# hendraet/synthesis-in-style

Measured on NVIDIA B200. Metric: labelled image pairs/sec at 256^2, higher is better.
Workload: dtype bf16x3 (3-term bf16 split, fp32 accumulate)

## Files before the change

### synthesis_in_style_b200/csrc/modconv_tc.cu

```cuda
#include <cuda.h>
#include <cstring>
#include "common.cuh"
#include "kernels.h"
#include "modconv_tc.h"

namespace sis {

using bf16 = __nv_bfloat16;

__device__ __forceinline__ uint32_t smem_u32(const void* p) { return (uint32_t)__cvta_generic_to_shared(p); }

__device__ __forceinline__ bool elect_one() {
    uint32_t pred;
    asm volatile("{\n\t.reg .pred P;\n\telect.sync _|P, 0xffffffff;\n\tselp.u32 %0, 1, 0, P;\n\t}" : "=r"(pred));
    return pred != 0;
}

__device__ __forceinline__ void mbar_init(uint64_t* bar, uint32_t count) {
    asm volatile("mbarrier.init.shared::cta.b64 [%0], %1;" ::"r"(smem_u32(bar)), "r"(count) : "memory");
}
__device__ __forceinline__ void mbar_expect_tx(uint64_t* bar, uint32_t bytes, uint32_t pred = 1u) {
    asm volatile("{\n\t.reg .pred q;\n\tsetp.ne.b32 q, %2, 0;\n\t@q mbarrier.arrive.expect_tx.shared::cta.b64 _, [%0], %1;\n\t}"
                 ::"r"(smem_u32(bar)), "r"(bytes), "r"(pred) : "memory");
}
// ... 671 lines not shown
template <int BN, int BK, bool UP4>
__global__ void __launch_bounds__(TC_THREADS, 1)
modconv_tc_halo_rw_kernel(const __grid_constant__ TcMaps maps, const __grid_constant__ TcKernelArgs a) {
    using Cfg = TcHaloRwCfg<BN, BK, UP4>;
    constexpr int NA = Cfg::NA, ROW = Cfg::ROW;
    extern __shared__ uint8_t smem_raw[];
    uint8_t* smem_w = (uint8_t*)(((uintptr_t)smem_raw + 1023) & ~(uintptr_t)1023);
    uint8_t* smem_a = smem_w + Cfg::W_BYTES;
    uint64_t* bars = (uint64_t*)(smem_a + NA * Cfg::A_STAGE);
    uint64_t* afull_bar = bars;
    uint64_t* aempty_bar = bars + NA;
    uint64_t* tfull_bar = bars + 2 * NA;
    uint64_t* tempty_bar = tfull_bar + 2;
    uint64_t* wfull_bar = tempty_bar + 2;
    uint32_t* tmem_ptr_smem = (uint32_t*)(wfull_bar + 1);

    const int warp = __shfl_sync(0xffffffffu, (int)(threadIdx.x >> 5), 0), lane = threadIdx.x & 31;
    const int unit0 = (int)blockIdx.x, unit_stride = (int)gridDim.x;
    if (warp == 0 && lane == 0) {
        tma_prefetch_desc(&maps.a[0][0]); tma_prefetch_desc(&maps.a[0][1]);
        tma_prefetch_desc(&maps.w[0]); tma_prefetch_desc(&maps.w[1]);
        for (int i = 0; i < NA; ++i) { mbar_init(&afull_bar[i], 1); mbar_init(&aempty_bar[i], 1); }
        for (int i = 0; i < 2; ++i) { mbar_init(&tfull_bar[i], 1); mbar_init(&tempty_bar[i], TC_EPI_WARPS); }
        mbar_init(wfull_bar, 1);
        asm volatile("fence.mbarrier_init.release.cluster;" ::: "memory");
    }
    if (warp == 1) {
        asm volatile("tcgen05.alloc.cta_group::1.sync.aligned.shared::cta.b32 [%0], %1;" ::"r"(smem_u32(tmem_ptr_smem)), "r"((uint32_t)Cfg::TMEM_COLS) : "memory");
        asm volatile("tcgen05.relinquish_alloc_permit.cta_group::1.sync.aligned;" ::: "memory");
    }
    tc_fence_before();
    __syncthreads();
    tc_fence_after();
    const uint32_t tmem_base = *tmem_ptr_smem;
    const TcSubProblem& s = a.sub[0];

    if (warp == 0) {
        if (elect_one()) {
            mbar_expect_tx(wfull_bar, Cfg::W_BYTES);
            for (int tap = 0; tap < 9; ++tap) {
                tma_load_3d(&maps.w[0], wfull_bar, smem_w + tap * Cfg::W_TAP, 0, 0, s.widx[tap]);
                tma_load_3d(&maps.w[1], wfull_bar, smem_w + tap * Cfg::W_TAP + Cfg::W_TILE, 0, 0, s.widx[tap]);
            }
        }
        __syncwarp();
        int as = 0; uint32_t aphase = 0;
        for (int t = unit0; t < a.total_tiles; t += unit_stride) {
            const TileCoord c = decode_tile<BN, true, 1>(a, t, 0);
            mbar_wait(&aempty_bar[as], aphase ^ 1, a.error, 0x500 + as);
            uint8_t* sa = smem_a + as * Cfg::A_STAGE;
            if (elect_one()) {
                mbar_expect_tx(&afull_bar[as], 2 * Cfg::A_BYTES);
                tma_load_4d(&maps.a[0][0], &afull_bar[as], sa, 0, c.x0 - 1, c.y0 - 1, c.b0);
                tma_load_4d(&maps.a[0][1], &afull_bar[as], sa + Cfg::A_PAD, 0, c.x0 - 1, c.y0 - 1, c.b0);
            }
            __syncwarp();
            if (++as == NA) { as = 0; aphase ^= 1; }
        }
    } else if (warp == 1) {
        constexpr uint32_t idesc = (1u << 4) | (1u << 7) | (1u << 10) | ((uint32_t)(BN >> 3) << 17) | ((uint32_t)(BM >> 4) << 24);
        int as = 0; uint32_t aphase = 0;
        int acc = 0; uint32_t acc_phase = 0;
        mbar_wait(wfull_bar, 0, a.error, 0x700);
        const uint32_t sw0 = smem_u32(smem_w);
        for (int t = unit0; t < a.total_tiles; t += unit_stride) {
            mbar_wait(&tempty_bar[acc], acc_phase ^ 1, a.error, 0x200 + acc);
            mbar_wait(&afull_bar[as], aphase, a.error, 0x600 + as);
            tc_fence_after();
            const uint32_t d_tile = tmem_base + (uint32_t)(acc * Cfg::ACC_COLS);
            const uint32_t sa = smem_u32(smem_a + as * Cfg::A_STAGE);
            if (elect_one()) {
                uint32_t started = 0;
#pragma unroll 1
                for (int tap = 0; tap < 9; ++tap) {
                    const uint32_t aoff = (uint32_t)(((s.dy[tap] + 1) * HALO_W + (s.dx[tap] + 1)) * ROW);
                    const uint64_t d_ah = make_halo_desc<ROW>(sa + aoff), d_al = make_halo_desc<ROW>(sa + Cfg::A_PAD + aoff);
                    const uint32_t sb = sw0 + (uint32_t)(tap * Cfg::W_TAP);
                    const uint64_t d_bh = make_smem_desc<ROW>(sb), d_bl = make_smem_desc<ROW>(sb + Cfg::W_TILE);
                    const int ph = UP4 ? s.phase[tap] : 0;
                    const uint32_t d_tmem = d_tile + (uint32_t)(ph * BN);
                    const uint32_t fresh = UP4 ? (((started >> ph) & 1u) ^ 1u) : (tap ? 0u : 1u);
                    started |= 1u << ph;
#pragma unroll
                    for (int k = 0; k < BK / UMMA_K; ++k) {
                        const uint64_t koff = (uint64_t)((k * UMMA_K * 2) >> 4);
                        umma_bf16(d_tmem, d_ah + koff, d_bh + koff, idesc, (fresh && k == 0) ? 0u : 1u);
                        umma_bf16(d_tmem, d_ah + koff, d_bl + koff, idesc, 1u);
                        umma_bf16(d_tmem, d_al + koff, d_bh + koff, idesc, 1u);
                    }
                }
                umma_commit(&aempty_bar[as]);
                umma_commit(&tfull_bar[acc]);
            }
            __syncwarp();
            if (++as == NA) { as = 0; aphase ^= 1; }
            if (++acc == 2) { acc = 0; acc_phase ^= 1; }
        }
    } else {
        tc_epilogue<BN, true, 1, UP4>(a, tfull_bar, tempty_bar, tmem_base, 0, warp, lane, unit0, unit_stride);
    }
    tc_fence_before();
    __syncthreads();
    if (warp == 1) {
        __syncwarp();
        tc_fence_after();
        asm volatile("tcgen05.dealloc.cta_group::1.sync.aligned.b32 %0, %1;" ::"r"(tmem_base), "r"((uint32_t)Cfg::TMEM_COLS) : "memory");
    }
}

constexpr int HT_TH = 32, HT_TW = 8, HT_W = HT_TW + 2, HT_H = HT_TH + 2, HT_BK = 32, HT_N = HT_TH * HT_TW;
struct TcHaloTCfg {
    static constexpr int ROW = HT_BK * 2;
    static constexpr int A_BYTES = HT_H * HT_W * ROW;
    static constexpr int A_PAD = (A_BYTES + 1023) / 1024 * 1024;
    static constexpr int A_STAGE = 2 * A_PAD;
    static constexpr int NA = 2;
    static constexpr int W_TILE_BYTES = 128 * ROW;
    static constexpr int W_STAGE = 2 * W_TILE_BYTES;
    static constexpr int NW = 8;
    static constexpr int SMEM_BYTES = NA * A_STAGE + NW * W_STAGE + 1024 + 512;
    static constexpr int TMEM_COLS = 512;
};

__device__ __forceinline__ uint64_t make_halo_t_desc(uint32_t saddr) {
    uint64_t d = 0;
    d |= (uint64_t)((saddr >> 4) & 0x3FFF);
    d |= (uint64_t)1 << 16;
    d |= (uint64_t)((HT_W * TcHaloTCfg::ROW) >> 4) << 32;
    d |= (uint64_t)1 << 46;
    d |= (uint64_t)4 << 61;
    return d;
}

__global__ void __launch_bounds__(TC_THREADS, 1)
modconv_tc_halo_t_kernel(const __grid_constant__ TcMaps maps, const __grid_constant__ TcKernelArgs a) {
    using Cfg = TcHaloTCfg;
    constexpr int NA = Cfg::NA, NW = Cfg::NW, BK = HT_BK;
    extern __shared__ uint8_t smem_raw[];
    uint8_t* smem = (uint8_t*)(((uintptr_t)smem_raw + 1023) & ~(uintptr_t)1023);
    uint8_t* smem_w = smem + NA * Cfg::A_STAGE;
    uint64_t* bars = (uint64_t*)(smem_w + NW * Cfg::W_STAGE);
    uint64_t* full_bar = bars;
    uint64_t* empty_bar = bars + NW;
    uint64_t* afull_bar = bars + 2 * NW;
    uint64_t* aempty_bar = bars + 2 * NW + NA;
    uint64_t* tfull_bar = bars + 2 * NW + 2 * NA;
    uint64_t* tempty_bar = tfull_bar + 2;
    uint32_t* tmem_ptr_smem = (uint32_t*)(tempty_bar + 2);

    const int warp = __shfl_sync(0xffffffffu, (int)(threadIdx.x >> 5), 0), lane = threadIdx.x & 31;
    const int tiles_x = a.sub[0].ow / HT_TW, tiles_y = a.sub[0].oh / HT_TH;
    const int m_tiles = a.batch * tiles_y * tiles_x;
    const int per = a.nsub;

    if (warp == 0 && lane == 0) {
        tma_prefetch_desc(&maps.a[0][0]); tma_prefetch_desc(&maps.a[0][1]);
        tma_prefetch_desc(&maps.w[0]); tma_prefetch_desc(&maps.w[1]);
        for (int i = 0; i < NW; ++i) { mbar_init(&full_bar[i], 1); mbar_init(&empty_bar[i], 1); }
        for (int i = 0; i < NA; ++i) { mbar_init(&afull_bar[i], 1); mbar_init(&aempty_bar[i], 1); }
        for (int i = 0; i < 2; ++i) { mbar_init(&tfull_bar[i], 1); mbar_init(&tempty_bar[i], TC_EPI_WARPS); }
        asm volatile("fence.mbarrier_init.release.cluster;" ::: "memory");
    }
    if (warp == 1) {
        asm volatile("tcgen05.alloc.cta_group::1.sync.aligned.shared::cta.b32 [%0], %1;" ::"r"(smem_u32(tmem_ptr_smem)), "r"((uint32_t)Cfg::TMEM_COLS) : "memory");
        asm volatile("tcgen05.relinquish_alloc_permit.cta_group::1.sync.aligned;" ::: "memory");
    }
    tc_fence_before();
    __syncthreads();
    tc_fence_after();
    const uint32_t tmem_base = *tmem_ptr_smem;

    if (warp == 0) {
        {
            int as = 0; uint32_t aphase = 0;
            int ws = 0; uint32_t wphase = 0;
            for (int t = blockIdx.x; t < a.total_tiles; t += gridDim.x) {
                const int rt = t % (m_tiles * per), n0 = (t / (m_tiles * per)) * 128;
                const int m = rt / per;
                const TcSubProblem& s = a.sub[per == 1 ? 0 : ((rt % per) + m) & 3];
                const int x0 = (m % tiles_x) * HT_TW, y0 = ((m / tiles_x) % tiles_y) * HT_TH, b = m / (tiles_x * tiles_y);
                for (int kc = 0; kc < a.kchunks; ++kc) {
                    mbar_wait(&aempty_bar[as], aphase ^ 1, a.error, 0x500 + as);
                    uint8_t* sa = smem + as * Cfg::A_STAGE;
                    if (elect_one()) {
                        mbar_expect_tx(&afull_bar[as], 2 * Cfg::A_BYTES);
                        tma_load_4d(&maps.a[0][0], &afull_bar[as], sa, kc * BK, x0 - 1, y0 - 1, b);
                        tma_load_4d(&maps.a[0][1], &afull_bar[as], sa + Cfg::A_PAD, kc * BK, x0 - 1, y0 - 1, b);
                    }
                    __syncwarp();
                    if (++as == NA) { as = 0; aphase ^= 1; }
                    for (int tap = 0; tap < s.ntaps; ++tap) {
                        mbar_wait(&empty_bar[ws], wphase ^ 1, a.error, 0x100 + ws);
                        uint8_t* sw = smem_w + ws * Cfg::W_STAGE;
                        if (elect_one()) {
                            mbar_expect_tx(&full_bar[ws], Cfg::W_STAGE);
                            tma_load_3d(&maps.w[0], &full_bar[ws], sw, kc * BK, n0, s.widx[tap]);
                            tma_load_3d(&maps.w[1], &full_bar[ws], sw + Cfg::W_TILE_BYTES, kc * BK, n0, s.widx[tap]);
                        }
                        __syncwarp();
                        if (++ws == NW) { ws = 0; wphase ^= 1; }
                    }
                }
            }
        }
    } else if (warp == 1) {
        {
            constexpr uint32_t idesc = (1u << 4) | (1u << 7) | (1u << 10) | ((uint32_t)(HT_N >> 3) << 17) | ((uint32_t)(128 >> 4) << 24);
            int as = 0; uint32_t aphase = 0;
            int ws = 0; uint32_t wphase = 0;
            int acc = 0; uint32_t acc_phase = 0;
            for (int t = blockIdx.x; t < a.total_tiles; t += gridDim.x) {
                const int rt = t % (m_tiles * per);
                const TcSubProblem& s = a.sub[per == 1 ? 0 : ((rt % per) + rt / per) & 3];
                mbar_wait(&tempty_bar[acc], acc_phase ^ 1, a.error, 0x200 + acc);
                tc_fence_after();
                const uint32_t d_tmem = tmem_base + (uint32_t)(acc * HT_N);
                for (int kc = 0; kc < a.kchunks; ++kc) {
                    mbar_wait(&afull_bar[as], aphase, a.error, 0x600 + as);
                    const uint32_t sa = smem_u32(smem + as * Cfg::A_STAGE);
                    for (int tap = 0; tap < s.ntaps; ++tap) {
                        mbar_wait(&full_bar[ws], wphase, a.error, 0x300 + ws);
                        tc_fence_after();
                        const uint32_t xoff = (uint32_t)(((s.dy[tap] + 1) * HT_W + (s.dx[tap] + 1)) * Cfg::ROW);
                        const uint64_t d_xh = make_halo_t_desc(sa + xoff), d_xl = make_halo_t_desc(sa + Cfg::A_PAD + xoff);
                        const uint32_t sw = smem_u32(smem_w + ws * Cfg::W_STAGE);
                        const uint64_t d_wh = make_smem_desc<Cfg::ROW>(sw), d_wl = make_smem_desc<Cfg::ROW>(sw + Cfg::W_TILE_BYTES);
                        if (elect_one()) {
#pragma unroll
                            for (int k = 0; k < BK / UMMA_K; ++k) {
                                const uint64_t koff = (uint64_t)((k * UMMA_K * 2) >> 4);
                                umma_bf16(d_tmem, d_wh + koff, d_xh + koff, idesc, (kc | tap | k) ? 1u : 0u);
                                umma_bf16(d_tmem, d_wl + koff, d_xh + koff, idesc, 1u);
                                umma_bf16(d_tmem, d_wh + koff, d_xl + koff, idesc, 1u);
                            }
                            umma_commit(&empty_bar[ws]);
                            if (tap == s.ntaps - 1) {
                                umma_commit(&aempty_bar[as]);
                                if (kc == a.kchunks - 1) umma_commit(&tfull_bar[acc]);
                            }
                        }
                        __syncwarp();
                        if (++ws == NW) { ws = 0; wphase ^= 1; }
                    }
                    if (++as == NA) { as = 0; aphase ^= 1; }
                }
                if (++acc == 2) { acc = 0; acc_phase ^= 1; }
            }
        }
    } else {
        const int quarter = warp & 3;
        const int chalf = (warp - 2) >> 2;
        int acc = 0; uint32_t acc_phase = 0;
        for (int t = blockIdx.x; t < a.total_tiles; t += gridDim.x) {
            const int rt = t % (m_tiles * per), n0 = (t / (m_tiles * per)) * 128;
            const int m = rt / per;
            const TcSubProblem& s = a.sub[per == 1 ? 0 : ((rt % per) + m) & 3];
            const int x0 = (m % tiles_x) * HT_TW, y0 = ((m / tiles_x) % tiles_y) * HT_TH, b = m / (tiles_x * tiles_y);
            const int ch = n0 + quarter * 32 + lane;
            const float d = __ldg(a.demod + (int64_t)b * a.cout + ch);
            const float bias = a.bias ? __ldg(a.bias + ch) : 0.0f;
            const float sn = a.s_next ? __ldg(a.s_next + (int64_t)b * a.cout + ch) : 0.0f;
            float* plane = a.out_f32 + ((int64_t)b * a.cout + ch) * ((int64_t)a.out_h * a.out_w);
            const float* nzp = a.noise ? a.noise + (int64_t)b * a.noise_bstride : nullptr;
            mbar_wait(&tfull_bar[acc], acc_phase, a.error, 0x400 + acc);
            tc_fence_after();
            const uint32_t taddr = tmem_base + ((uint32_t)(quarter * 32) << 16) + (uint32_t)(acc * HT_N);
#pragma unroll 1
            for (int c0 = chalf * 32; c0 < HT_N; c0 += 64) {
                uint32_t r[32];
                tmem_ld_32x32(taddr + (uint32_t)c0, r);
                tmem_ld_wait();
                if (a.mode == 1) {
#pragma unroll
                    for (int rr = 0; rr < 4; ++rr) {
                        const int oy = (y0 + c0 / HT_TW + rr) * s.ostride + s.ooff_y;
                        float* row = a.out_f32 + (((int64_t)b * a.out_h + oy) * a.out_w + x0 * s.ostride + s.ooff_x) * a.cout + ch;
#pragma unroll
                        for (int j = 0; j < 8; ++j) row[(int64_t)j * s.ostride * a.cout] = __fmul_rn(__uint_as_float(r[rr * 8 + j]), d);
                    }
                    continue;
                }
#pragma unroll
                for (int rr = 0; rr < 4; ++rr) {
                    const int y = y0 + c0 / HT_TW + rr;
                    float nz[8] = {0.f, 0.f, 0.f, 0.f, 0.f, 0.f, 0.f, 0.f};
                    if (nzp) {
                        const float4 n0v = __ldg(reinterpret_cast<const float4*>(nzp + (int64_t)y * a.out_w + x0));
                        const float4 n1v = __ldg(reinterpret_cast<const float4*>(nzp + (int64_t)y * a.out_w + x0) + 1);
                        nz[0] = n0v.x; nz[1] = n0v.y; nz[2] = n0v.z; nz[3] = n0v.w; nz[4] = n1v.x; nz[5] = n1v.y; nz[6] = n1v.z; nz[7] = n1v.w;
                    }
                    float v[8];
#pragma unroll
                    for (int j = 0; j < 8; ++j) {
                        float x = __fmul_rn(__uint_as_float(r[rr * 8 + j]), d);
                        x = __fadd_rn(x, __fmul_rn(a.noise_w, nz[j]));
                        if (a.bias) x = __fadd_rn(x, bias);
                        if (a.act) x = lrelu_scale(x, 0.2f, 1.41421356237309504880f);
                        v[j] = x;
                    }
                    float4* dst = reinterpret_cast<float4*>(plane + (int64_t)y * a.out_w + x0);
                    dst[0] = make_float4(v[0], v[1], v[2], v[3]);
                    dst[1] = make_float4(v[4], v[5], v[6], v[7]);
                    if (a.s_next) {
                        const int64_t off = (((int64_t)b * a.out_h + y) * a.out_w + x0) * a.cout + (ch & ~1);
#pragma unroll
                        for (int j = 0; j < 8; ++j) {
                            const float xs = __fmul_rn(v[j], sn);
                            const float other = __shfl_xor_sync(0xffffffffu, xs, 1);
                            if ((j & 1) == (lane & 1)) {
                                const float c0v = (lane & 1) ? other : xs, c1v = (lane & 1) ? xs : other;
                                const bf16 h0 = __float2bfloat16_rn(c0v), h1 = __float2bfloat16_rn(c1v);
                                const bf16 l0 = __float2bfloat16_rn(c0v - __bfloat162float(h0)), l1 = __float2bfloat16_rn(c1v - __bfloat162float(h1));
                                *reinterpret_cast<uint32_t*>(a.next_hi + off + (int64_t)j * a.cout) =
                                    (uint32_t)__bfloat16_as_ushort(h0) | ((uint32_t)__bfloat16_as_ushort(h1) << 16);
                                *reinterpret_cast<uint32_t*>(a.next_lo + off + (int64_t)j * a.cout) =
                                    (uint32_t)__bfloat16_as_ushort(l0) | ((uint32_t)__bfloat16_as_ushort(l1) << 16);
                            }
                        }
                    }
                }
            }
            tc_fence_before();
            __syncwarp();
            if (lane == 0) mbar_arrive(&tempty_bar[acc]);
            if (++acc == 2) { acc = 0; acc_phase ^= 1; }
        }
    }
    tc_fence_before();
    __syncthreads();
    if (warp == 1) {
        __syncwarp();
        tc_fence_after();
        asm volatile("tcgen05.dealloc.cta_group::1.sync.aligned.b32 %0, %1;" ::"r"(tmem_base), "r"((uint32_t)Cfg::TMEM_COLS) : "memory");
    }
}

struct BlurSplitArgs {
    const float* in; int IH, IW;
    float* out_f32; int OH, OW, C, batch;
    const float* blur_k; const float* noise; int64_t noise_bstride; float noise_w; const float* bias;
    const float* s_next; bf16* next_hi; bf16* next_lo;
    int act;
};
constexpr int BS_TH = 8, BS_IH = BS_TH + 3;
template <int CB> struct BlurGeo {
    static constexpr int LPG = CB / 2;
    static constexpr int GROUPS = 32 / LPG;
    static constexpr int TW = 8 * GROUPS * 2;
    static constexpr int IW = TW + 3;
    static constexpr int OPITCH = BS_TH * TW + 1;
    static constexpr int SMEM = BS_IH * IW * CB * 4;
    static_assert(CB * OPITCH * 4 <= SMEM, "the transposed output must fit in the input tile");
};

using u64 = unsigned long long;
__device__ __forceinline__ float2 ffma2(float2 a, float2 b, float2 c) {
    float2 d;
    asm("fma.rn.f32x2 %0, %1, %2, %3;" : "=l"(reinterpret_cast<u64&>(d)) : "l"(reinterpret_cast<u64&>(a)), "l"(reinterpret_cast<u64&>(b)), "l"(reinterpret_cast<u64&>(c)));
    return d;
}
__device__ __forceinline__ float2 fmul2(float2 a, float2 b) {
    float2 d;
    asm("mul.rn.f32x2 %0, %1, %2;" : "=l"(reinterpret_cast<u64&>(d)) : "l"(reinterpret_cast<u64&>(a)), "l"(reinterpret_cast<u64&>(b)));
    return d;
}
__device__ __forceinline__ float2 fadd2(float2 a, float2 b) {
    float2 d;
    asm("add.rn.f32x2 %0, %1, %2;" : "=l"(reinterpret_cast<u64&>(d)) : "l"(reinterpret_cast<u64&>(a)), "l"(reinterpret_cast<u64&>(b)));
    return d;
}
__device__ __forceinline__ float2 splat2(float v) { return make_float2(v, v); }
__device__ __forceinline__ float2 lds_f2(uint32_t addr) {
    float2 v;
    asm volatile("ld.shared.v2.f32 {%0, %1}, [%2];" : "=f"(v.x), "=f"(v.y) : "r"(addr));
    return v;
}
__device__ __forceinline__ float lds_f1(uint32_t addr) {
    float v;
    asm volatile("ld.shared.f32 %0, [%1];" : "=f"(v) : "r"(addr));
    return v;
}
__device__ __forceinline__ void sts_f1(uint32_t addr, float v) { asm volatile("st.shared.f32 [%0], %1;" ::"r"(addr), "f"(v) : "memory"); }

template <bool SEP, int CB>
__global__ void __launch_bounds__(256, 2) blur_act_split_kernel(BlurSplitArgs a, const __grid_constant__ CUtensorMap in_map) {
    using G = BlurGeo<CB>;
    constexpr int TW = G::TW, IW = G::IW, LPG = G::LPG, OPITCH = G::OPITCH, TILE_BYTES = G::SMEM;
    extern __shared__ __align__(128) float stile_raw[];
    __shared__ float sk[16], skx[4], sky[4];
    __shared__ float snz[BS_TH * TW];
    __shared__ uint64_t tma_bar[2];
    float* const ring0 = (float*)(((uintptr_t)stile_raw + 127) & ~(uintptr_t)127);
    const int tid = threadIdx.x, lane = tid & 31, warp = tid >> 5;
    const int grp = lane / LPG, cl = lane - grp * LPG;
    if (tid < 16) sk[tid] = a.blur_k[(3 - tid / 4) * 4 + (3 - tid % 4)];
    __syncthreads();
    if (tid < 4) { sky[tid] = sk[tid * 4]; skx[tid] = SEP ? sk[tid] / sk[0] : 0.0f; }
    const int tiles_x = (a.OW + TW - 1) / TW, tiles_y = (a.OH + BS_TH - 1) / BS_TH;
    const int cgroups = (a.C + CB - 1) / CB;
    const int64_t total = (int64_t)a.batch * tiles_y * tiles_x * cgroups;
    auto tile_coords = [&](int64_t tile, int& b, int& y0, int& x0, int& c0) {
        const int cg = (int)(tile % cgroups);
        int64_t r = tile / cgroups;
        const int tx = (int)(r % tiles_x); r /= tiles_x;
        const int ty = (int)(r % tiles_y);
        b = (int)(r / tiles_y); y0 = ty * BS_TH; x0 = tx * TW; c0 = cg * CB;
    };
    if (tid == 0) {
        mbar_init(&tma_bar[0], 1); mbar_init(&tma_bar[1], 1);
        asm volatile("fence.mbarrier_init.release.cluster;" ::: "memory");
        if ((int64_t)blockIdx.x < total) {
            int b, y0, x0, c0;
            tile_coords(blockIdx.x, b, y0, x0, c0);
            mbar_expect_tx(&tma_bar[0], TILE_BYTES);
            tma_load_4d(&in_map, &tma_bar[0], ring0, c0, x0 - 1, y0 - 1, b);
        }
    }
    int it = 0;
    for (int64_t tile = blockIdx.x; tile < total; tile += gridDim.x, ++it) {
        int b, y0, x0, c0;
        tile_coords(tile, b, y0, x0, c0);
        float* const stile = ring0 + (it & 1) * (TILE_BYTES / 4);
        const uint32_t stile_u32 = smem_u32(stile);
        __syncthreads();
        if (tid == 0 && tile + gridDim.x < total) {
            int nb, ny0, nx0, nc0;
            tile_coords(tile + gridDim.x, nb, ny0, nx0, nc0);
            asm volatile("fence.proxy.async.shared::cta;" ::: "memory");
            mbar_expect_tx(&tma_bar[(it + 1) & 1], TILE_BYTES);
            tma_load_4d(&in_map, &tma_bar[(it + 1) & 1], ring0 + ((it + 1) & 1) * (TILE_BYTES / 4), nc0, nx0 - 1, ny0 - 1, nb);
        }
        if (tid < BS_TH * TW) {
            const int oy = y0 + tid / TW, ox = x0 + tid % TW;
            snz[tid] = (a.noise && oy < a.OH && ox < a.OW) ? a.noise_w * __ldg(a.noise + (int64_t)b * a.noise_bstride + (int64_t)oy * a.OW + ox) : 0.0f;
        }
        mbar_wait(&tma_bar[it & 1], (uint32_t)((it >> 1) & 1), nullptr, 0);
        __syncthreads();

        float2 res[2][BS_TH];
        const int px = (warp * G::GROUPS + grp) * 2;
        const uint32_t in_base = stile_u32 + (uint32_t)(px * LPG + cl) * 8u;
        {
            const bool chok = c0 + 2 * cl < a.C;
            const float2 bias = (chok && a.bias) ? *reinterpret_cast<const float2*>(a.bias + c0 + 2 * cl) : make_float2(0.f, 0.f);
            const float2 sn = (a.s_next && chok) ? *reinterpret_cast<const float2*>(a.s_next + (int64_t)b * a.C + c0 + 2 * cl) : make_float2(0.f, 0.f);
            const bool colok0 = chok && x0 + px < a.OW, colok1 = chok && x0 + px + 1 < a.OW;
            const int64_t off0 = (((int64_t)b * a.OH + y0) * a.OW + x0 + px) * a.C + c0 + 2 * cl;
            __nv_bfloat162* ph = reinterpret_cast<__nv_bfloat162*>(a.next_hi + off0);
            __nv_bfloat162* pl = reinterpret_cast<__nv_bfloat162*>(a.next_lo + off0);
            const int c2 = a.C >> 1;
            const int64_t rs2 = ((int64_t)a.OW * a.C) >> 1;
            const bool st0 = a.s_next != nullptr && colok0, st1 = a.s_next != nullptr && colok1;
            float2 win[2][4][SEP ? 1 : 4];
#pragma unroll
            for (int rr = 0; rr < BS_IH; ++rr) {
                float2 in5[5];
#pragma unroll
                for (int j = 0; j < 5; ++j) in5[j] = lds_f2(in_base + (uint32_t)((rr * IW + j) * LPG) * 8u);
#pragma unroll
                for (int cx = 0; cx < 2; ++cx) {
#pragma unroll
                    for (int ky = 0; ky < 3; ++ky)
#pragma unroll
                        for (int kx = 0; kx < (SEP ? 1 : 4); ++kx) win[cx][ky][kx] = win[cx][ky + 1][kx];
                    if (SEP) {
                        float2 h = make_float2(0.f, 0.f);
#pragma unroll
                        for (int kx = 0; kx < 4; ++kx) h = ffma2(in5[cx + kx], splat2(skx[kx]), h);
                        win[cx][3][0] = h;
                    } else {
#pragma unroll
                        for (int kx = 0; kx < 4; ++kx) win[cx][3][kx] = in5[cx + kx];
                    }
                }
                if (rr >= 3) {
                    const int py = rr - 3;
                    const bool rowok = y0 + py < a.OH;
#pragma unroll
// ... 320 lines not shown
    for (int ky = py; ky < 3; ky += 2)
        for (int kx = px; kx < 3; kx += 2) {
            s.dy[s.ntaps] = (short)(y0 - ky / 2); s.dx[s.ntaps] = (short)(x0 - kx / 2);
            s.widx[s.ntaps] = (signed char)(ky * 3 + kx); s.phase[s.ntaps] = (signed char)(py * 2 + px); s.ntaps++;
        }
}

static void set_im2col_runs(TcSubProblem& s, int batch) {
    s.m_tiles = (int)ceil_div64((int64_t)batch * s.oh * s.ow, BM);
    s.base_dy = s.dy[0]; s.base_dx = s.dx[0];
    for (int t = 1; t < s.ntaps; ++t) { s.base_dy = std::min<int>(s.base_dy, s.dy[t]); s.base_dx = std::min<int>(s.base_dx, s.dx[t]); }
}

static TcKernelArgs conv_args(const TcWorkspace& ws, const TcConvCall& call, int BK) {
    TcKernelArgs a;
    memset(&a, 0, sizeof(a));
    const int H = call.res_in;
    a.batch = call.batch; a.cin = call.cin; a.cout = call.cout; a.kchunks = call.cin / BK; a.b_tiles = call.batch;
    a.demod = call.demod; a.error = ws.d_error;
    if (call.up) {
        a.mode = 1;
        a.out_f32 = call.upconv_tmp; a.out_h = 2 * H + 1; a.out_w = 2 * H + 1;
    } else {
        a.mode = 0; a.act = call.act ? 1 : 0;
        a.noise = call.noise; a.noise_bstride = call.noise_bstride; a.noise_w = call.noise_w; a.bias = call.bias;
        a.out_f32 = call.out_f32; a.out_h = H; a.out_w = H;
        a.s_next = call.s_next; a.next_hi = (bf16*)ws.a_hi[call.out_slot]; a.next_lo = (bf16*)ws.a_lo[call.out_slot];
    }
    return a;
}

template <auto Kernel, int SMEM_BYTES, int CG = 1>
static int launch_persistent(const TcMaps& maps, const TcKernelArgs& a, cudaStream_t stream) {
    static bool configured = false;
    if (!configured) {
        SIS_CHECK_CUDA(cudaFuncSetAttribute(Kernel, cudaFuncAttributeMaxDynamicSharedMemorySize, SMEM_BYTES));
        configured = true;
    }
    cudaLaunchConfig_t cfg;
    memset(&cfg, 0, sizeof(cfg));
    cfg.gridDim = dim3(a.total_tiles * CG < kNumSMs ? a.total_tiles * CG : kNumSMs);
    cfg.blockDim = dim3(TC_THREADS); cfg.dynamicSmemBytes = SMEM_BYTES; cfg.stream = stream;
    cudaLaunchAttribute attr[1];
    attr[0].id = cudaLaunchAttributeClusterDimension;
    attr[0].val.clusterDim.x = CG; attr[0].val.clusterDim.y = 1; attr[0].val.clusterDim.z = 1;
    cfg.attrs = attr; cfg.numAttrs = 1;
    SIS_CHECK_CUDA(cudaLaunchKernelEx(&cfg, Kernel, maps, a));
    SIS_CHECK_LAUNCH();
    return SIS_OK;
}

template <int BK, int CG>
static int launch_tc(int BN, const TcMaps& maps, const TcKernelArgs& a, cudaStream_t stream) {
    if (BN == 256) return launch_persistent<modconv_tc_kernel<256, BK, CG>, TcCfg<256, BK, CG>::SMEM_BYTES, CG>(maps, a, stream);
    if (BN == 128) return launch_persistent<modconv_tc_kernel<128, BK, CG>, TcCfg<128, BK, CG>::SMEM_BYTES, CG>(maps, a, stream);
    if (BN == 64) return launch_persistent<modconv_tc_kernel<64, BK, CG>, TcCfg<64, BK, CG>::SMEM_BYTES, CG>(maps, a, stream);
    if constexpr (CG == 1) {
        if (BN == 32) return launch_persistent<modconv_tc_kernel<32, BK, 1>, TcCfg<32, BK, 1>::SMEM_BYTES>(maps, a, stream);
    }
    set_error("tc_modconv: no per-tap kernel for BN %d with CG %d", BN, CG);
    return SIS_ERR_UNSUPPORTED;
}

template <int CG>
static int launch_tc_halo(int BN, int BK, const TcMaps& maps, const TcKernelArgs& a, cudaStream_t stream) {
    if (BK == 32) {
        if (BN == 64) return launch_persistent<modconv_tc_halo_kernel<64, CG, 32, false>, TcHaloCfg<64, CG, 32, false>::SMEM_BYTES, CG>(maps, a, stream);
        if constexpr (CG == 1) {
            if (BN == 32) return launch_persistent<modconv_tc_halo_kernel<32, 1, 32, false>, TcHaloCfg<32, 1, 32, false>::SMEM_BYTES>(maps, a, stream);
        }
    } else {
        if (BN == 256) return launch_persistent<modconv_tc_halo_kernel<256, CG, 64, false>, TcHaloCfg<256, CG, 64, false>::SMEM_BYTES, CG>(maps, a, stream);
        if (BN == 128) return launch_persistent<modconv_tc_halo_kernel<128, CG, 64, false>, TcHaloCfg<128, CG, 64, false>::SMEM_BYTES, CG>(maps, a, stream);
        if (BN == 64) return launch_persistent<modconv_tc_halo_kernel<64, CG, 64, false>, TcHaloCfg<64, CG, 64, false>::SMEM_BYTES, CG>(maps, a, stream);
        if constexpr (CG == 1) {
            if (BN == 32) return launch_persistent<modconv_tc_halo_kernel<32, 1, 64, false>, TcHaloCfg<32, 1, 64, false>::SMEM_BYTES>(maps, a, stream);
        }
    }
    set_error("tc_modconv: no halo kernel for BN %d, BK %d with CG %d", BN, BK, CG);
    return SIS_ERR_UNSUPPORTED;
}

static int launch_tc_halo_up4(int BN, int BK, int CG, const TcMaps& maps, const TcKernelArgs& a, cudaStream_t stream) {
    if (BN == 64 && CG == 2) {
        if (BK == 64) return launch_persistent<modconv_tc_halo_kernel<64, 2, 64, true>, TcHaloCfg<64, 2, 64, true>::SMEM_BYTES, 2>(maps, a, stream);
        return launch_persistent<modconv_tc_halo_kernel<64, 2, 32, true>, TcHaloCfg<64, 2, 32, true>::SMEM_BYTES, 2>(maps, a, stream);
    }
    if (BN == 64) {
        if (BK == 64) return launch_persistent<modconv_tc_halo_kernel<64, 1, 64, true>, TcHaloCfg<64, 1, 64, true>::SMEM_BYTES>(maps, a, stream);
        return launch_persistent<modconv_tc_halo_kernel<64, 1, 32, true>, TcHaloCfg<64, 1, 32, true>::SMEM_BYTES>(maps, a, stream);
    }
    if (BK == 64) return launch_persistent<modconv_tc_halo_kernel<32, 1, 64, true>, TcHaloCfg<32, 1, 64, true>::SMEM_BYTES>(maps, a, stream);
    return launch_persistent<modconv_tc_halo_kernel<32, 1, 32, true>, TcHaloCfg<32, 1, 32, true>::SMEM_BYTES>(maps, a, stream);
}

template <int CB>
static int launch_blur_split(const BlurSplitArgs& bs, bool sep, cudaStream_t stream) {
    using G = BlurGeo<CB>;
    static int blocks_per_sm[2] = {0, 0};
    const size_t smem = 2 * (size_t)G::SMEM + 128;
    auto kern = sep ? blur_act_split_kernel<true, CB> : blur_act_split_kernel<false, CB>;
    int& bps = blocks_per_sm[sep ? 1 : 0];
    if (!bps) {
        SIS_CHECK_CUDA(cudaFuncSetAttribute(kern, cudaFuncAttributeMaxDynamicSharedMemorySize, (int)smem));
        SIS_CHECK_CUDA(cudaOccupancyMaxActiveBlocksPerMultiprocessor(&bps, kern, 256, smem));
        if (bps < 1) bps = 1;
    }
    CUtensorMap in_map;
    memset(&in_map, 0, sizeof(in_map));
    const uint64_t dims[4] = {(uint64_t)bs.C, (uint64_t)bs.IW, (uint64_t)bs.IH, (uint64_t)bs.batch};
    const uint32_t box[4] = {(uint32_t)CB, (uint32_t)G::IW, (uint32_t)BS_IH, 1};
    SIS_PROPAGATE(make_map_f32(&in_map, bs.in, 4, dims, box));
    const int64_t total = (int64_t)bs.batch * ceil_div(bs.OH, BS_TH) * ceil_div(bs.OW, G::TW) * ceil_div(bs.C, CB);
    const int grid = (int)std::min<int64_t>(total, (int64_t)kNumSMs * bps);
    ProfScope prof(PROF_BLUR_SPLIT, stream);
    kern<<<grid, 256, smem, stream>>>(bs, in_map);
    SIS_CHECK_LAUNCH();
    return SIS_OK;
}

static int tc_blur_after_upconv(TcWorkspace& ws, const TcConvCall& call, cudaStream_t stream) {
    const int B = call.batch, H = call.res_in;
    BlurSplitArgs bs;
    bs.in = call.upconv_tmp; bs.IH = 2 * H + 1; bs.IW = 2 * H + 1;
    bs.out_f32 = call.out_f32; bs.OH = call.res_out; bs.OW = call.res_out; bs.C = call.cout; bs.batch = B;
    bs.blur_k = call.blur_k; bs.noise = call.noise; bs.noise_bstride = call.noise_bstride; bs.noise_w = call.noise_w; bs.bias = call.bias;
    bs.s_next = call.s_next; bs.next_hi = (bf16*)ws.a_hi[call.out_slot]; bs.next_lo = (bf16*)ws.a_lo[call.out_slot];
    bs.act = call.act ? 1 : 0;
    SIS_REQUIRE(bs.C % 32 == 0, "tc_modconv: the blur pass needs Cout %% 32 == 0 (got %d)", bs.C);
    if (bs.C % 64 != 0 && bs.OW >= 32) return launch_blur_split<32>(bs, call.blur_separable, stream);
    return launch_blur_split<64>(bs, call.blur_separable, stream);
}

int tc_modconv(TcWorkspace& ws, const TcConvWeights& w, const TcConvCall& call, cudaStream_t stream) {
    const int conv_cat = call.cout <= 64 ? PROF_CONV_TC_NARROW : PROF_CONV_TC;
    SIS_REQUIRE(w.hi && w.cin == call.cin && w.cout == call.cout, "tc_modconv: weights not packed for this layer");
    const int B = call.batch, H = call.res_in;
    if (!call.up && call.cout == 128 && call.cin % HT_BK == 0 && H % HT_TH == 0) {
        TcKernelArgs a = conv_args(ws, call, HT_BK);
        a.nsub = 1;
        TcSubProblem& s = a.sub[0];
        set_conv_taps(s);
        s.oh = H; s.ow = H; s.ostride = 1;
        a.total_tiles = B * (H / HT_TH) * (H / HT_TW);
        TcMaps maps;
        memset(&maps, 0, sizeof(maps));
        SIS_PROPAGATE(make_halo_maps(maps, ws, call, HT_BK, HT_W, HT_H));
        SIS_PROPAGATE(make_weight_maps(maps, w.hi, w.lo, call.cin, call.cout, 9, HT_BK, 128));
        ProfScope prof(conv_cat, stream);
        return launch_persistent<modconv_tc_halo_t_kernel, TcHaloTCfg::SMEM_BYTES>(maps, a, stream);
    }
    if (call.up && call.cout == 128 && call.cin % 64 == 0 && H % HT_TH == 0 && H <= 128 ) {
        TcKernelArgs a = conv_args(ws, call, HT_BK);
        a.nsub = 4;
        for (int p = 0; p < 4; ++p) {
            TcSubProblem& s = a.sub[p];
            add_phase_taps(s, p >> 1, p & 1);
            s.oh = H; s.ow = H; s.ostride = 2; s.ooff_y = p >> 1; s.ooff_x = p & 1;
        }
        a.total_tiles = B * (H / HT_TH) * (H / HT_TW) * 4;
        TcMaps maps;
        memset(&maps, 0, sizeof(maps));
        SIS_PROPAGATE(make_halo_maps(maps, ws, call, HT_BK, HT_W, HT_H));
        SIS_PROPAGATE(make_weight_maps(maps, w.hi, w.lo, call.cin, call.cout, 9, HT_BK, 128));
        {
            ProfScope prof(conv_cat, stream);
            SIS_PROPAGATE((launch_persistent<modconv_tc_halo_t_kernel, TcHaloTCfg::SMEM_BYTES>(maps, a, stream)));
        }
        TcKernelArgs b = conv_args(ws, call, 64);
        b.nsub = 4;
        struct Strip { int py, px, y0, x0, oh, ow; };
        const Strip strips[4] = {{0, 0, H, 0, 1, H + 1}, {0, 1, H, 0, 1, H}, {0, 0, 0, H, H, 1}, {1, 0, 0, H, H, 1}};
        TcMaps mb;
        memset(&mb, 0, sizeof(mb));
        int tiles = 0;
        for (int i = 0; i < 4; ++i) {
            const Strip& sp = strips[i];
            TcSubProblem& s = b.sub[i];
            add_phase_taps(s, sp.py, sp.px, sp.y0, sp.x0);
            s.oh = sp.oh; s.ow = sp.ow; s.ostride = 2; s.ooff_y = 2 * sp.y0 + sp.py; s.ooff_x = 2 * sp.x0 + sp.px;
            set_im2col_runs(s, B);
            s.tile_begin = tiles;
            tiles += s.m_tiles;
            SIS_PROPAGATE(make_im2col_maps(mb, i, s, ws, call, 64));
        }
        b.total_tiles = tiles;
        SIS_PROPAGATE(make_weight_maps(mb, w.hi, w.lo, call.cin, call.cout, 9, 64, 128));
        {
            ProfScope prof(conv_cat, stream);
            SIS_PROPAGATE((launch_tc<64, 1>(128, mb, b, stream)));
        }
        return tc_blur_after_upconv(ws, call, stream);
    }
    if (call.up && (call.cout == 64 || call.cout == 32) && call.cin % 32 == 0 && H >= 8) {
        const int BN = call.cout, BK = call.cin % 64 == 0 ? 64 : 32;
        TcKernelArgs a = conv_args(ws, call, BK);
        a.nsub = 1;
        TcSubProblem& s = a.sub[0];
        for (int p = 0; p < 4; ++p) add_phase_taps(s, p >> 1, p & 1);
        s.oh = H + 1; s.ow = H + 1; s.ostride = 2;
        s.tiles_y = ceil_div(H + 1, HALO_TH); s.tiles_x = ceil_div(H + 1, HALO_TW);
        const int64_t m_tiles = (int64_t)B * s.tiles_y * s.tiles_x;
        const int CG = (BN == 64 && m_tiles >= 2 * kNumSMs) ? 2 : 1;
        a.total_tiles = (int)ceil_div64(m_tiles, CG);
        TcMaps maps;
        memset(&maps, 0, sizeof(maps));
        SIS_PROPAGATE(make_halo_maps(maps, ws, call, BK, HALO_W, HALO_H));
        SIS_PROPAGATE(make_weight_maps(maps, w.hi, w.lo, call.cin, call.cout, 9, BK, BN / CG));
        {
            ProfScope prof(conv_cat, stream);
            if (BN == 32 && BK == 64 && a.kchunks == 1)
                SIS_PROPAGATE((launch_persistent<modconv_tc_halo_rw_kernel<32, 64, true>, TcHaloRwCfg<32, 64, true>::SMEM_BYTES>(maps, a, stream)));
            else
                SIS_PROPAGATE(launch_tc_halo_up4(BN, BK, CG, maps, a, stream));
        }
        return tc_blur_after_upconv(ws, call, stream);
    }
    const bool halo = !call.up && H >= HALO_TH && H % HALO_TH == 0 && (call.cin % 64 == 0 || (call.cin % 32 == 0 && call.cout <= 64));
    const int BK = call.cin % 64 == 0 ? 64 : 32;
    SIS_REQUIRE(call.cin % BK == 0, "tc_modconv: Cin must be a multiple of 32 (got %d)", call.cin);
    SIS_REQUIRE(call.cout % 32 == 0, "tc_modconv: Cout must be a multiple of 32 (got %d)", call.cout);
    const int64_t m_tiles_all = halo ? (int64_t)B * ceil_div(H, HALO_TH) * ceil_div(H, HALO_TW)
                                     : ceil_div64((int64_t)B * (call.up ? (2 * H + 1) * (2 * H + 1) : H * H), BM);
    int BN = 32;
    for (int cand = 256; cand >= 32; cand /= 2) {
        if (call.cout % cand) continue;
        if (m_tiles_all * (call.cout / cand) >= kNumSMs || cand == 32) { BN = cand; break; }
    }
    if (!call.up && !halo && m_tiles_all * (call.cout / BN) < 4 * kNumSMs) {
        double best = 1e30;
        for (int cand = 256; cand >= 32; cand /= 2) {
            if (call.cout % cand) continue;
            const int64_t tiles_c = m_tiles_all * (call.cout / cand);
            const double waves = (double)((tiles_c + kNumSMs - 1) / kNumSMs);
            const double mma = 12.0 * std::max(cand / 2.0, (128.0 + cand) / 4.0);
            const double cost = waves * std::max(mma, (32768.0 + 256.0 * cand) / 60.0);
            if (cost < best) { best = cost; BN = cand; }
        }
    }
    SIS_REQUIRE(call.cout % BN == 0, "tc_modconv: unsupported Cout %d", call.cout);
    const int n_tiles = call.cout / BN;
    const int CG = (BN >= 64 && m_tiles_all * n_tiles >= 2 * kNumSMs) ? 2 : 1;

    TcKernelArgs a = conv_args(ws, call, BK);
    if (!call.up) {
        a.nsub = 1;
        TcSubProblem& s = a.sub[0];
        set_conv_taps(s);
        s.oh = H; s.ow = H; s.ostride = 1;
        if (halo) {
            s.tiles_y = ceil_div(H, HALO_TH); s.tiles_x = ceil_div(H, HALO_TW);
            a.total_tiles = ceil_div(B * s.tiles_y * s.tiles_x, CG) * n_tiles;
        } else {
            set_im2col_runs(s, B);
            a.total_tiles = ceil_div(s.m_tiles, CG) * n_tiles;
        }
    } else {
        a.nsub = 4;
        int umax = 0;
        for (int p = 0; p < 4; ++p) {
            TcSubProblem& s = a.sub[p];
            const int py = p >> 1, px = p & 1;
            add_phase_taps(s, py, px);
            s.oh = H + (py == 0 ? 1 : 0); s.ow = H + (px == 0 ? 1 : 0);
            s.ostride = 2; s.ooff_y = py; s.ooff_x = px;
            set_im2col_runs(s, B);
            umax = std::max(umax, ceil_div(s.m_tiles, CG));
        }
        a.interleave_units = umax;
        a.total_tiles = 4 * umax * n_tiles;
    }

    TcMaps maps;
    memset(&maps, 0, sizeof(maps));
    if (halo) SIS_PROPAGATE(make_halo_maps(maps, ws, call, BK, HALO_W, HALO_H));
    else
        for (int i = 0; i < a.nsub; ++i) SIS_PROPAGATE(make_im2col_maps(maps, i, a.sub[i], ws, call, BK));
    SIS_PROPAGATE(make_weight_maps(maps, w.hi, w.lo, call.cin, call.cout, 9, BK, BN / CG));
    {
        ProfScope prof(conv_cat, stream);
        if (halo && BN == 32 && BK == 32 && CG == 1 && a.kchunks == 1 && n_tiles == 1)
            SIS_PROPAGATE((launch_persistent<modconv_tc_halo_rw_kernel<32, 32, false>, TcHaloRwCfg<32, 32, false>::SMEM_BYTES>(maps, a, stream)));
        else if (halo)
            SIS_PROPAGATE(CG == 2 ? launch_tc_halo<2>(BN, BK, maps, a, stream) : launch_tc_halo<1>(BN, BK, maps, a, stream));
        else if (CG == 2)
            SIS_PROPAGATE((BK == 64 ? launch_tc<64, 2>(BN, maps, a, stream) : launch_tc<32, 2>(BN, maps, a, stream)));
        else
            SIS_PROPAGATE((BK == 64 ? launch_tc<64, 1>(BN, maps, a, stream) : launch_tc<32, 1>(BN, maps, a, stream)));
    }
    if (call.up) SIS_PROPAGATE(tc_blur_after_upconv(ws, call, stream));
    return SIS_OK;
}

int tc_nchw_to_nhwc_split(void* hi, void* lo, const float* x, int batch, int c, int64_t hw, int c_total, int c_off, cudaStream_t stream) {
    SIS_REQUIRE(c % 2 == 0 && c_off % 2 == 0 && c_total % 2 == 0, "nchw_to_nhwc_split: channel counts must be even");
    dim3 grid((unsigned)ceil_div64(hw, 64), (unsigned)ceil_div(c, 64), (unsigned)batch);
    ProfScope prof(PROF_OTHER, stream);
    nchw_to_nhwc_split_kernel<<<grid, 256, 0, stream>>>((bf16*)hi, (bf16*)lo, x, c, hw, c_total, c_off);
    SIS_CHECK_LAUNCH();
    return SIS_OK;
}

int tc_pack_matrix_split(void* hi, void* lo, const float* w, int n, int k, int k_total, int k_off, int out_total, int out_off, cudaStream_t stream) {
    const int64_t total = (int64_t)n * k;
    int grid = (int)std::min<int64_t>(ceil_div64(total, 256), (int64_t)kNumSMs * 8);
    pack_matrix_split_kernel<<<grid, 256, 0, stream>>>((bf16*)hi, (bf16*)lo, w, n, k, k_total, k_off, out_total, out_off);
    SIS_CHECK_LAUNCH();
    return SIS_OK;
}

int tc_conv1x1(const void* a_hi, const void* a_lo, const void* w_hi, const void* w_lo, int batch, int res, int cin, int cout,
               const float* ones, float* out, bool out_nhwc, unsigned int* d_error, cudaStream_t stream) {
    SIS_REQUIRE(cin % 32 == 0, "tc_conv1x1: K must be a multiple of 32 (got %d)", cin);
// ... 33 lines not shown
```

Before: 4035.

## Pair upsample phases per tile to share halo loads across two TMEM accumulators

The transposed-conv upsample path now groups the four output phases into two sub-problems, each holding two phases, so one halo A tile load feeds both phases. The MMA warp accumulates each phase into its own TMEM slot, and the epilogue drains both slots in turn. This halves the number of tiles and the A-operand TMA traffic per output. In exchange the double-buffered accumulator is used by both phases of the same tile, so the epilogue of one tile no longer overlaps the MMAs of the next. The change also relies on the per-tap s.phase field being filled by add_phase_taps.

```diff
diff --git a/synthesis_in_style_b200/csrc/modconv_tc.cu b/synthesis_in_style_b200/csrc/modconv_tc.cu
--- a/synthesis_in_style_b200/csrc/modconv_tc.cu
+++ b/synthesis_in_style_b200/csrc/modconv_tc.cu
@@ -847,6 +847,8 @@
     const int tiles_x = a.sub[0].ow / HT_TW, tiles_y = a.sub[0].oh / HT_TH;
     const int m_tiles = a.batch * tiles_y * tiles_x;
     const int per = a.nsub;
+    const bool pairs = a.mode == 1;
+    auto slot_of = [&](const TcSubProblem& s, int tap) { return (pairs && s.phase[tap] != s.phase[0]) ? 1 : 0; };
 
     if (warp == 0 && lane == 0) {
         tma_prefetch_desc(&maps.a[0][0]); tma_prefetch_desc(&maps.a[0][1]);
@@ -872,7 +874,7 @@
             for (int t = blockIdx.x; t < a.total_tiles; t += gridDim.x) {
                 const int rt = t % (m_tiles * per), n0 = (t / (m_tiles * per)) * 128;
                 const int m = rt / per;
-                const TcSubProblem& s = a.sub[per == 1 ? 0 : ((rt % per) + m) & 3];
+                const TcSubProblem& s = a.sub[((rt % per) + m) % per];
                 const int x0 = (m % tiles_x) * HT_TW, y0 = ((m / tiles_x) % tiles_y) * HT_TH, b = m / (tiles_x * tiles_y);
                 for (int kc = 0; kc < a.kchunks; ++kc) {
                     mbar_wait(&aempty_bar[as], aphase ^ 1, a.error, 0x500 + as);
@@ -903,19 +905,23 @@
             constexpr uint32_t idesc = (1u << 4) | (1u << 7) | (1u << 10) | ((uint32_t)(HT_N >> 3) << 17) | ((uint32_t)(128 >> 4) << 24);
             int as = 0; uint32_t aphase = 0;
             int ws = 0; uint32_t wphase = 0;
-            int acc = 0; uint32_t acc_phase = 0;
+            int acc0 = 0;
+            uint32_t acc_bits = 0u;
             for (int t = blockIdx.x; t < a.total_tiles; t += gridDim.x) {
                 const int rt = t % (m_tiles * per);
-                const TcSubProblem& s = a.sub[per == 1 ? 0 : ((rt % per) + rt / per) & 3];
-                mbar_wait(&tempty_bar[acc], acc_phase ^ 1, a.error, 0x200 + acc);
-                tc_fence_after();
-                const uint32_t d_tmem = tmem_base + (uint32_t)(acc * HT_N);
+                const TcSubProblem& s = a.sub[((rt % per) + rt / per) % per];
                 for (int kc = 0; kc < a.kchunks; ++kc) {
                     mbar_wait(&afull_bar[as], aphase, a.error, 0x600 + as);
                     const uint32_t sa = smem_u32(smem + as * Cfg::A_STAGE);
                     for (int tap = 0; tap < s.ntaps; ++tap) {
+                        const int slot = slot_of(s, tap);
+                        const int acc = pairs ? slot : acc0;
+                        const bool first = tap == 0 || slot_of(s, tap - 1) != slot;
+                        const bool last = tap == s.ntaps - 1 || slot_of(s, tap + 1) != slot;
+                        if (kc == 0 && first) mbar_wait(&tempty_bar[acc], ((acc_bits >> acc) & 1u) ^ 1u, a.error, 0x200 + acc);
                         mbar_wait(&full_bar[ws], wphase, a.error, 0x300 + ws);
                         tc_fence_after();
+                        const uint32_t d_tmem = tmem_base + (uint32_t)(acc * HT_N);
                         const uint32_t xoff = (uint32_t)(((s.dy[tap] + 1) * HT_W + (s.dx[tap] + 1)) * Cfg::ROW);
                         const uint64_t d_xh = make_halo_t_desc(sa + xoff), d_xl = make_halo_t_desc(sa + Cfg::A_PAD + xoff);
                         const uint32_t sw = smem_u32(smem_w + ws * Cfg::W_STAGE);
@@ -924,32 +930,32 @@
 #pragma unroll
                             for (int k = 0; k < BK / UMMA_K; ++k) {
                                 const uint64_t koff = (uint64_t)((k * UMMA_K * 2) >> 4);
-                                umma_bf16(d_tmem, d_wh + koff, d_xh + koff, idesc, (kc | tap | k) ? 1u : 0u);
+                                umma_bf16(d_tmem, d_wh + koff, d_xh + koff, idesc, (kc != 0 || !first || k != 0) ? 1u : 0u);
                                 umma_bf16(d_tmem, d_wl + koff, d_xh + koff, idesc, 1u);
                                 umma_bf16(d_tmem, d_wh + koff, d_xl + koff, idesc, 1u);
                             }
                             umma_commit(&empty_bar[ws]);
-                            if (tap == s.ntaps - 1) {
-                                umma_commit(&aempty_bar[as]);
-                                if (kc == a.kchunks - 1) umma_commit(&tfull_bar[acc]);
-                            }
+                            if (tap == s.ntaps - 1) umma_commit(&aempty_bar[as]);
+                            if (kc == a.kchunks - 1 && last) umma_commit(&tfull_bar[acc]);
                         }
                         __syncwarp();
                         if (++ws == NW) { ws = 0; wphase ^= 1; }
                     }
                     if (++as == NA) { as = 0; aphase ^= 1; }
                 }
-                if (++acc == 2) { acc = 0; acc_phase ^= 1; }
+                if (pairs) acc_bits ^= 3u;
+                else { acc_bits ^= 1u << acc0; acc0 ^= 1; }
             }
         }
     } else {
         const int quarter = warp & 3;
         const int chalf = (warp - 2) >> 2;
-        int acc = 0; uint32_t acc_phase = 0;
+        int acc0 = 0;
+        uint32_t acc_bits = 0u;
         for (int t = blockIdx.x; t < a.total_tiles; t += gridDim.x) {
             const int rt = t % (m_tiles * per), n0 = (t / (m_tiles * per)) * 128;
             const int m = rt / per;
-            const TcSubProblem& s = a.sub[per == 1 ? 0 : ((rt % per) + m) & 3];
+            const TcSubProblem& s = a.sub[((rt % per) + m) % per];
             const int x0 = (m % tiles_x) * HT_TW, y0 = ((m / tiles_x) % tiles_y) * HT_TH, b = m / (tiles_x * tiles_y);
             const int ch = n0 + quarter * 32 + lane;
             const float d = __ldg(a.demod + (int64_t)b * a.cout + ch);
@@ -957,68 +963,73 @@
             const float sn = a.s_next ? __ldg(a.s_next + (int64_t)b * a.cout + ch) : 0.0f;
             float* plane = a.out_f32 + ((int64_t)b * a.cout + ch) * ((int64_t)a.out_h * a.out_w);
             const float* nzp = a.noise ? a.noise + (int64_t)b * a.noise_bstride : nullptr;
-            mbar_wait(&tfull_bar[acc], acc_phase, a.error, 0x400 + acc);
-            tc_fence_after();
-            const uint32_t taddr = tmem_base + ((uint32_t)(quarter * 32) << 16) + (uint32_t)(acc * HT_N);
+            for (int i = 0; i < (pairs ? 2 : 1); ++i) {
+                const int acc = pairs ? i : acc0;
+                const int ph = i == 0 ? s.phase[0] : s.phase[s.ntaps - 1];
+                mbar_wait(&tfull_bar[acc], (acc_bits >> acc) & 1u, a.error, 0x400 + acc);
+                tc_fence_after();
+                const uint32_t taddr = tmem_base + ((uint32_t)(quarter * 32) << 16) + (uint32_t)(acc * HT_N);
 #pragma unroll 1
-            for (int c0 = chalf * 32; c0 < HT_N; c0 += 64) {
-                uint32_t r[32];
-                tmem_ld_32x32(taddr + (uint32_t)c0, r);
-                tmem_ld_wait();
-                if (a.mode == 1) {
+                for (int c0 = chalf * 32; c0 < HT_N; c0 += 64) {
+                    uint32_t r[32];
+                    tmem_ld_32x32(taddr + (uint32_t)c0, r);
+                    tmem_ld_wait();
+                    if (a.mode == 1) {
+#pragma unroll
+                        for (int rr = 0; rr < 4; ++rr) {
+                            const int oy = (y0 + c0 / HT_TW + rr) * 2 + (ph >> 1);
+                            float* row = a.out_f32 + (((int64_t)b * a.out_h + oy) * a.out_w + x0 * 2 + (ph & 1)) * a.cout + ch;
+#pragma unroll
+                            for (int j = 0; j < 8; ++j) row[(int64_t)j * 2 * a.cout] = __fmul_rn(__uint_as_float(r[rr * 8 + j]), d);
+                        }
+                        continue;
+                    }
 #pragma unroll
                     for (int rr = 0; rr < 4; ++rr) {
-                        const int oy = (y0 + c0 / HT_TW + rr) * s.ostride + s.ooff_y;
-                        float* row = a.out_f32 + (((int64_t)b * a.out_h + oy) * a.out_w + x0 * s.ostride + s.ooff_x) * a.cout + ch;
-#pragma unroll
-                        for (int j = 0; j < 8; ++j) row[(int64_t)j * s.ostride * a.cout] = __fmul_rn(__uint_as_float(r[rr * 8 + j]), d);
-                    }
-                    continue;
-                }
-#pragma unroll
-                for (int rr = 0; rr < 4; ++rr) {
-                    const int y = y0 + c0 / HT_TW + rr;
-                    float nz[8] = {0.f, 0.f, 0.f, 0.f, 0.f, 0.f, 0.f, 0.f};
-                    if (nzp) {
-                        const float4 n0v = __ldg(reinterpret_cast<const float4*>(nzp + (int64_t)y * a.out_w + x0));
-                        const float4 n1v = __ldg(reinterpret_cast<const float4*>(nzp + (int64_t)y * a.out_w + x0) + 1);
-                        nz[0] = n0v.x; nz[1] = n0v.y; nz[2] = n0v.z; nz[3] = n0v.w; nz[4] = n1v.x; nz[5] = n1v.y; nz[6] = n1v.z; nz[7] = n1v.w;
-                    }
-                    float v[8];
-#pragma unroll
-                    for (int j = 0; j < 8; ++j) {
-                        float x = __fmul_rn(__uint_as_float(r[rr * 8 + j]), d);
-                        x = __fadd_rn(x, __fmul_rn(a.noise_w, nz[j]));
-                        if (a.bias) x = __fadd_rn(x, bias);
-                        if (a.act) x = lrelu_scale(x, 0.2f, 1.41421356237309504880f);
-                        v[j] = x;
-                    }
-                    float4* dst = reinterpret_cast<float4*>(plane + (int64_t)y * a.out_w + x0);
-                    dst[0] = make_float4(v[0], v[1], v[2], v[3]);
-                    dst[1] = make_float4(v[4], v[5], v[6], v[7]);
-                    if (a.s_next) {
-                        const int64_t off = (((int64_t)b * a.out_h + y) * a.out_w + x0) * a.cout + (ch & ~1);
+                        const int y = y0 + c0 / HT_TW + rr;
+                        float nz[8] = {0.f, 0.f, 0.f, 0.f, 0.f, 0.f, 0.f, 0.f};
+                        if (nzp) {
+                            const float4 n0v = __ldg(reinterpret_cast<const float4*>(nzp + (int64_t)y * a.out_w + x0));
+                            const float4 n1v = __ldg(reinterpret_cast<const float4*>(nzp + (int64_t)y * a.out_w + x0) + 1);
+                            nz[0] = n0v.x; nz[1] = n0v.y; nz[2] = n0v.z; nz[3] = n0v.w; nz[4] = n1v.x; nz[5] = n1v.y; nz[6] = n1v.z; nz[7] = n1v.w;
+                        }
+                        float v[8];
 #pragma unroll
                         for (int j = 0; j < 8; ++j) {
-                            const float xs = __fmul_rn(v[j], sn);
-                            const float other = __shfl_xor_sync(0xffffffffu, xs, 1);
-                            if ((j & 1) == (lane & 1)) {
-                                const float c0v = (lane & 1) ? other : xs, c1v = (lane & 1) ? xs : other;
-                                const bf16 h0 = __float2bfloat16_rn(c0v), h1 = __float2bfloat16_rn(c1v);
-                                const bf16 l0 = __float2bfloat16_rn(c0v - __bfloat162float(h0)), l1 = __float2bfloat16_rn(c1v - __bfloat162float(h1));
-                                *reinterpret_cast<uint32_t*>(a.next_hi + off + (int64_t)j * a.cout) =
-                                    (uint32_t)__bfloat16_as_ushort(h0) | ((uint32_t)__bfloat16_as_ushort(h1) << 16);
-                                *reinterpret_cast<uint32_t*>(a.next_lo + off + (int64_t)j * a.cout) =
-                                    (uint32_t)__bfloat16_as_ushort(l0) | ((uint32_t)__bfloat16_as_ushort(l1) << 16);
+                            float x = __fmul_rn(__uint_as_float(r[rr * 8 + j]), d);
+                            x = __fadd_rn(x, __fmul_rn(a.noise_w, nz[j]));
+                            if (a.bias) x = __fadd_rn(x, bias);
+                            if (a.act) x = lrelu_scale(x, 0.2f, 1.41421356237309504880f);
+                            v[j] = x;
+                        }
+                        float4* dst = reinterpret_cast<float4*>(plane + (int64_t)y * a.out_w + x0);
+                        dst[0] = make_float4(v[0], v[1], v[2], v[3]);
+                        dst[1] = make_float4(v[4], v[5], v[6], v[7]);
+                        if (a.s_next) {
+                            const int64_t off = (((int64_t)b * a.out_h + y) * a.out_w + x0) * a.cout + (ch & ~1);
+#pragma unroll
+                            for (int j = 0; j < 8; ++j) {
+                                const float xs = __fmul_rn(v[j], sn);
+                                const float other = __shfl_xor_sync(0xffffffffu, xs, 1);
+                                if ((j & 1) == (lane & 1)) {
+                                    const float c0v = (lane & 1) ? other : xs, c1v = (lane & 1) ? xs : other;
+                                    const bf16 h0 = __float2bfloat16_rn(c0v), h1 = __float2bfloat16_rn(c1v);
+                                    const bf16 l0 = __float2bfloat16_rn(c0v - __bfloat162float(h0)), l1 = __float2bfloat16_rn(c1v - __bfloat162float(h1));
+                                    *reinterpret_cast<uint32_t*>(a.next_hi + off + (int64_t)j * a.cout) =
+                                        (uint32_t)__bfloat16_as_ushort(h0) | ((uint32_t)__bfloat16_as_ushort(h1) << 16);
+                                    *reinterpret_cast<uint32_t*>(a.next_lo + off + (int64_t)j * a.cout) =
+                                        (uint32_t)__bfloat16_as_ushort(l0) | ((uint32_t)__bfloat16_as_ushort(l1) << 16);
+                                }
                             }
                         }
                     }
                 }
+                tc_fence_before();
+                __syncwarp();
+                if (lane == 0) mbar_arrive(&tempty_bar[acc]);
+                acc_bits ^= 1u << acc;
             }
-            tc_fence_before();
-            __syncwarp();
-            if (lane == 0) mbar_arrive(&tempty_bar[acc]);
-            if (++acc == 2) { acc = 0; acc_phase ^= 1; }
+            if (!pairs) acc0 ^= 1;
         }
     }
     tc_fence_before();
@@ -1645,13 +1656,14 @@
     }
     if (call.up && call.cout == 128 && call.cin % 64 == 0 && H % HT_TH == 0 && H <= 128 ) {
         TcKernelArgs a = conv_args(ws, call, HT_BK);
-        a.nsub = 4;
-        for (int p = 0; p < 4; ++p) {
-            TcSubProblem& s = a.sub[p];
-            add_phase_taps(s, p >> 1, p & 1);
-            s.oh = H; s.ow = H; s.ostride = 2; s.ooff_y = p >> 1; s.ooff_x = p & 1;
-        }
-        a.total_tiles = B * (H / HT_TH) * (H / HT_TW) * 4;
+        a.nsub = 2;
+        for (int i = 0; i < 2; ++i) {
+            TcSubProblem& s = a.sub[i];
+            add_phase_taps(s, 0, i);
+            add_phase_taps(s, 1, 1 - i);
+            s.oh = H; s.ow = H; s.ostride = 2;
+        }
+        a.total_tiles = B * (H / HT_TH) * (H / HT_TW) * 2;
         TcMaps maps;
         memset(&maps, 0, sizeof(maps));
         SIS_PROPAGATE(make_halo_maps(maps, ws, call, HT_BK, HT_W, HT_H));
```

New measurement: 3932, median of 6. 0.974x the previous value.
